# SonyCSLParis/audio-metrics

Hardware: AMD Instinct MI355X
Metric: evaluate() embeddings/sec (FAD+KD+PRDC), 2×100k CLAP-512 sets, 1/2/4/8 GPUs (higher is better)
Workload: dtype f32

## Files before the change

### audio-metrics_amd/csrc/pairwise_common.h

```cpp
#pragma once
#include "am_common.h"
#include "tile_engine.h"
#include <stdlib.h>

namespace am {

constexpr int EV_DEFAULT = EV_RSRC | EV_FRAGDB | EV_EARLY;
constexpr int WIDE_TILE_ROWS = 256;

#ifdef AM_DEV_KNOBS
static int env_int(const char* name, int dflt) {
    const char* v = getenv(name);
    return v ? atoi(v) : dflt;
}
static int engine_variant() {
    static const int v = env_int("AM_ENGINE_VARIANT", EV_DEFAULT);
    return v;
}
#else
static constexpr int env_int(const char*, int dflt) { return dflt; }
static constexpr int engine_variant() { return EV_DEFAULT; }
#endif

struct WorkItem {
// ... 141 lines not shown
}

constexpr unsigned FAST_COUNTED = 0x80000000u;
constexpr unsigned FAST_BOTH = 0x80000000u;
constexpr int FAST_ROW_OVERFLOW = 0x40000000;
constexpr unsigned FAST_HOLE = 0xffffffffu;

__device__ __forceinline__ unsigned long long lanes_le(float a, float b) { return __builtin_amdgcn_fcmpf(a, b, 5); }
__device__ __forceinline__ unsigned long long lanes_ge(float a, float b) { return __builtin_amdgcn_fcmpf(a, b, 3); }
__device__ __forceinline__ unsigned long long lanes_lt(float a, float b) { return __builtin_amdgcn_fcmpf(a, b, 4); }

template <int KCAP, class Lane = LaneInfo, int TBX = TB, int MT = 2>
struct KnnFastEpilogue {
    static constexpr int NWAVES = TBX == WIDE_TILE_ROWS ? 8 : 4;
    static constexpr int NT = Lane::NT;
    static constexpr bool ACC_INIT = Lane::ACC_INIT;
    const float* qnorm;
    const float* thr;
    int64_t n, pblock;
    float* aux;
    uint2* wgq;
    float* wgv;
    int wq;
    int wcap;
    uint2* shq;
    float* shv;
    int* qn;
    int shcap;
    uint2* ovq;
    float* ovv;
// ... 37 lines not shown
    }
    __device__ __forceinline__ void aux_issue(int, int64_t qtile) {
        if (L.tid < TBX) {
            const int64_t j = qtile * TBX + L.tid;
            aux_n = j < n ? qnorm[j] : INFINITY;
            aux_t = j < n ? __hip_atomic_load(thr + j, __ATOMIC_RELAXED, __HIP_MEMORY_SCOPE_AGENT) : -INFINITY;
        }
    }
    __device__ __forceinline__ void aux_commit(int t) {
        if (L.tid < TBX) {
            aux[(t & 1) * 2 * TBX + L.tid] = ACC_INIT ? aux_n * idsc : aux_n;
            aux[(t & 1) * 2 * TBX + TBX + L.tid] = ACC_INIT ? aux_t * idsc : aux_t;
        }
    }
    __device__ __forceinline__ f32x16 acc_init(int t, int mt) const {
        const float* a = aux + (t & 1) * 2 * TBX + L.wm * (MT * 32) + L.h * 4 + mt * 32;
        f32x16 c;
#pragma unroll
        for (int g4 = 0; g4 < 4; ++g4) {
            const f32x4 v = *reinterpret_cast<const f32x4*>(a + g4 * 8);
            c[g4 * 4 + 0] = v.x; c[g4 * 4 + 1] = v.y; c[g4 * 4 + 2] = v.z; c[g4 * 4 + 3] = v.w;
        }
        return c;
    }
    __device__ __forceinline__ void finish(int t, int64_t qtile, f32x16 (&acc)[MT][NT]) {
        const float* a = aux + (t & 1) * 2 * TBX + L.wm * (MT * 32) + L.h * 4;
        const bool mirror = qtile != pblock;
#ifdef AM_DEV_KNOBS
        if constexpr (TBX == WIDE_TILE_ROWS) {
            if (g_wide_dbg & 2) return;
        }
#endif
        const unsigned jbase = (unsigned)(qtile * TBX) + L.wm * (MT * 32) + L.h * 4;
        if constexpr (ACC_INIT) {
            float xsm[NT];
#pragma unroll
            for (int nt = 0; nt < NT; ++nt) xsm[nt] = mirror ? xs[nt] : INFINITY;
#pragma unroll
            for (int mt = 0; mt < MT; ++mt) {
                f32x4 tqs[4];
#pragma unroll
                for (int g4 = 0; g4 < 4; ++g4) tqs[g4] = *reinterpret_cast<const f32x4*>(a + TBX + mt * 32 + g4 * 8);
#pragma unroll
                for (int nt = 0; nt < NT; ++nt) {
                    float amax4[4], wmax4[4];
#pragma unroll
                    for (int g4 = 0; g4 < 4; ++g4) {
                        float am = -INFINITY, wm = -INFINITY;
#pragma unroll
                        for (int e = 0; e < 4; ++e) {
                            am = fmaxf(am, acc[mt][nt][g4 * 4 + e]);
                            wm = fmaxf(wm, acc[mt][nt][g4 * 4 + e] - tqs[g4][e]);
                        }
                        amax4[g4] = am;
                        wmax4[g4] = wm;
                    }
                    const float amax = fmaxf(fmaxf(amax4[0], amax4[1]), fmaxf(amax4[2], amax4[3]));
// ... 8 lines not shown
#endif
#pragma unroll
                    for (int g4 = 0; g4 < 4; ++g4) {
                        if ((lanes_le(fmaf(dsc, amax4[g4], xn[nt]), pl) | lanes_ge(wmax4[g4], xsm[nt])) == 0ull) continue;
#pragma unroll
                        for (int e = 0; e < 4; ++e) {
                            const int reg = g4 * 4 + e;
                            const float u = fmaf(dsc, acc[mt][nt][reg], xn[nt]);
                            const float w = acc[mt][nt][reg] - tqs[g4][e];
                            const unsigned long long sel = lanes_le(u, pl) | lanes_ge(w, xsm[nt]);
                            if (sel != 0ull) {
                                const bool own = u <= pl, mir = w >= xsm[nt];
                                const int below = __builtin_amdgcn_mbcnt_hi((unsigned)(sel >> 32), __builtin_amdgcn_mbcnt_lo((unsigned)sel, 0u));
                                const int slot = wq + below;
                                wq += __popcll(sel);
                                const unsigned j = jbase + mt * 32 + g4 * 8 + e;
#ifdef AM_DEV_KNOBS
                                if (TBX == WIDE_TILE_ROWS && (g_wide_dbg & 32)) continue;
#endif
                                if (own || mir) store_entry(slot, own ? prow[nt] : j, own ? j : prow[nt], own && mir, u);
                            }
                        }
                    }
                    const float vmin = tmin <= pl ? fmaxf(tmin, 0.f) : INFINITY;
#ifdef AM_DEV_KNOBS
                    if (TBX == WIDE_TILE_ROWS && (g_wide_dbg & 64)) continue;
#endif
                    if (lanes_lt(vmin, best[nt][KCAP - 1]) != 0ull) list_insert<KCAP>(best[nt], vmin);
                }
            }
            return;
        }
        const float mthr = mirror ? 0.f : -INFINITY;
#pragma unroll
        for (int mt = 0; mt < MT; ++mt) {
            f32x4 yn[4], tq[4];
#pragma unroll
            for (int g4 = 0; g4 < 4; ++g4) {
                yn[g4] = *reinterpret_cast<const f32x4*>(a + mt * 32 + g4 * 8);
                tq[g4] = *reinterpret_cast<const f32x4*>(a + TBX + mt * 32 + g4 * 8);
            }
#pragma unroll
            for (int nt = 0; nt < NT; ++nt) {
                float tmin4[4], marg4[4];
#pragma unroll
                for (int g4 = 0; g4 < 4; ++g4) {
                    float tm = INFINITY, mg = INFINITY;
#pragma unroll
                    for (int e = 0; e < 4; ++e) {
                        const float t = fmaf(dsc, acc[mt][nt][g4 * 4 + e], yn[g4][e]);
                        tm = fminf(tm, t);
                        mg = fminf(mg, t - tq[g4][e]);
                    }
                    tmin4[g4] = tm + xn[nt];
                    marg4[g4] = mg + xn[nt];
// ... 8 lines not shown
                }
#endif
#pragma unroll
                for (int g4 = 0; g4 < 4; ++g4) {
                    if ((lanes_le(tmin4[g4], pl) | lanes_le(marg4[g4], mthr)) == 0ull) continue;
#pragma unroll
                    for (int e = 0; e < 4; ++e) {
                        const int reg = g4 * 4 + e;
                        const float u = fmaf(dsc, acc[mt][nt][reg], xn[nt] + yn[g4][e]);
                        const bool own = u <= pl, mir = mirror && u <= tq[g4][e];
                        const unsigned long long sel = lanes_le(u, pl) | (mirror ? lanes_le(u, tq[g4][e]) : 0ull);
                        if (sel != 0ull) {
                            const int below = __builtin_amdgcn_mbcnt_hi((unsigned)(sel >> 32), __builtin_amdgcn_mbcnt_lo((unsigned)sel, 0u));
                            const int slot = wq + below;
                            wq += __popcll(sel);
                            const unsigned j = jbase + mt * 32 + g4 * 8 + e;
#ifdef AM_DEV_KNOBS
                            if (TBX == WIDE_TILE_ROWS && (g_wide_dbg & 32)) continue;
#endif
                            if (own || mir) store_entry(slot, own ? prow[nt] : j, own ? j : prow[nt], own && mir, u);
                        }
                    }
                }
                const float vmin = tmin <= pl ? fmaxf(tmin, 0.f) : INFINITY;
#ifdef AM_DEV_KNOBS
                if (TBX == WIDE_TILE_ROWS && (g_wide_dbg & 64)) continue;
#endif
                if (lanes_lt(vmin, best[nt][KCAP - 1]) != 0ull) list_insert<KCAP>(best[nt], vmin);
            }
        }
    }
// ... 38 lines not shown
```

### audio-metrics_amd/csrc/pairwise_pstat.hip

```cpp
#include "wide_kernels.h"
#include "pstat_engine.h"

namespace am {

template <int KSLABS>
struct PstatEng {
    using Lane = PLane;
    static constexpr int LDS_WORDS = pstat_lds_words(KSLABS);
    template <class TileMap, class Epi>
    static __device__ __forceinline__ void run(const float* Q, int64_t nq, int64_t ldq, const TileMap& tm, const float* P, int64_t np,
                                               int64_t ldp, int64_t prow0, int ntiles, int, float* lds, Lane& L, Epi& epi) {
        pstat_pipeline<KSLABS>(Q, nq, ldq, tm, P, np, ldp, prow0, ntiles, lds, L, epi);
    }
};

template <int KSLABS>
struct Pstat64Eng {
    using Lane = P64Lane;
    static constexpr int LDS_WORDS = pstat64_lds_words();
    template <class TileMap, class Epi>
    static __device__ __forceinline__ void run(const float* Q, int64_t nq, int64_t ldq, const TileMap& tm, const float* P, int64_t np,
                                               int64_t ldp, int64_t prow0, int ntiles, int, float* lds, Lane& L, Epi& epi) {
        pstat64_pipeline<KSLABS>(Q, nq, ldq, tm, P, np, ldp, prow0, ntiles, lds, L, epi);
    }
};

template <int KSLABS, bool WANT_MIN>
__global__ void __launch_bounds__(PTHREADS, 1)
cross_pstat_kernel(const float* __restrict__ Rb, int64_t Nr, int64_t ldr, const float* __restrict__ rnorm,
                   const float* __restrict__ rthr, const float* __restrict__ Cb, int64_t Nc, int64_t ldc,
                   const float* __restrict__ cnorm, const float* __restrict__ cthr, int Dh, int nchunks, int grp_rows,
                   const unsigned* __restrict__ maxn, unsigned* __restrict__ rmin_approx, unsigned* __restrict__ row_any,
                   unsigned* __restrict__ row_cover, int32_t* __restrict__ col_count, uint2* __restrict__ wgq, int qcap,
                   int* __restrict__ wgq_count, uint2* __restrict__ items, uint2* __restrict__ ovq, int* __restrict__ ov_count,
                   int ovcap, int* __restrict__ fail, float fc) {
    cross_wide_body<PstatEng<KSLABS>, WANT_MIN>(Rb, Nr, ldr, rnorm, rthr, Cb, Nc, ldc, cnorm, cthr, Dh, nchunks, grp_rows, maxn, rmin_approx,
                                                row_any, row_cover, col_count, wgq, qcap, wgq_count, items, ovq, ov_count, ovcap, fail, fc);
}

template <int KSLABS, int KCAP>
__global__ void __launch_bounds__(PTHREADS, 1)
knn_pstat_kernel(const float* __restrict__ Xb, int64_t N, int64_t ldh, const float* __restrict__ xnorm, float* thr, int Dh,
                 int win_tiles, int nwin, int per_win, int k1, const unsigned* __restrict__ maxn, float* __restrict__ partial,
                 int* __restrict__ cnt, int cap, uint2* __restrict__ wgq, float* __restrict__ wgv, int qcap,
                 int* __restrict__ wgq_count, int part, int nparts, float fc, uint2* __restrict__ ovq, float* __restrict__ ovv,
                 unsigned long long* __restrict__ ovn, int ovcap, const int* __restrict__ skip, int* __restrict__ region_counter) {
    knn_wide_body<PstatEng<KSLABS>, KCAP>(Xb, N, ldh, xnorm, thr, Dh, win_tiles, nwin, per_win, k1, maxn, partial, cnt, cap, wgq, wgv, qcap,
                                          wgq_count, part, nparts, fc, ovq, ovv, ovn, ovcap, skip, region_counter);
}

template <int KSLABS, bool WANT_MIN>
__global__ void __launch_bounds__(P64_THREADS, 2)
cross_pstat64_kernel(const float* __restrict__ Rb, int64_t Nr, int64_t ldr, const float* __restrict__ rnorm,
                     const float* __restrict__ rthr, const float* __restrict__ Cb, int64_t Nc, int64_t ldc,
                     const float* __restrict__ cnorm, const float* __restrict__ cthr, int Dh, int nchunks, int grp_rows,
                     const unsigned* __restrict__ maxn, unsigned* __restrict__ rmin_approx, unsigned* __restrict__ row_any,
                     unsigned* __restrict__ row_cover, int32_t* __restrict__ col_count, uint2* __restrict__ wgq, int qcap,
                     int* __restrict__ wgq_count, uint2* __restrict__ items, uint2* __restrict__ ovq, int* __restrict__ ov_count,
                     int ovcap, int* __restrict__ fail, float fc) {
    cross_wide_body<Pstat64Eng<KSLABS>, WANT_MIN>(Rb, Nr, ldr, rnorm, rthr, Cb, Nc, ldc, cnorm, cthr, Dh, nchunks, grp_rows, maxn, rmin_approx,
                                                  row_any, row_cover, col_count, wgq, qcap, wgq_count, items, ovq, ov_count, ovcap, fail, fc);
}
// ... 36 lines not shown
    AM_HIP_TRY(set_pstat_dev_symbols(st));
#endif
    hipLaunchKernelGGL((cross_pstat64_kernel<KSLABS, WANT_MIN>), dim3(blocks), dim3(P64_THREADS), lds_bytes, st, Rb, Nr, ldr, rnorm, rthr, Cb,
                       Nc, ldc, cnorm, cthr, Dh, nchunks, grp_rows, maxn, rmin_approx, row_any, row_cover, col_count, wgq, qcap,
                       wgq_count, items, ovq, ov_count, ovcap, fail, fc);
    AM_LAUNCH_CHECK();
    return AM_OK;
}

template <int KSLABS, bool WANT_MIN>
static int launch_cross_pstat_t(unsigned blocks, const float* Rb, int64_t Nr, int64_t ldr, const float* rnorm, const float* rthr,
                                const float* Cb, int64_t Nc, int64_t ldc, const float* cnorm, const float* cthr, int Dh, int nchunks,
                                int grp_rows, const unsigned* maxn, unsigned* rmin_approx, unsigned* row_any, unsigned* row_cover,
                                int32_t* col_count, uint2* wgq, int qcap, int* wgq_count, uint2* items, uint2* ovq, int* ov_count,
                                int ovcap, int* fail, float fc, hipStream_t st) {
    constexpr size_t lds_bytes = wide_cross_lds_bytes<PstatEng<KSLABS>>();
    AM_HIP_TRY(ensure_dynamic_lds(reinterpret_cast<const void*>(&cross_pstat_kernel<KSLABS, WANT_MIN>), (int)lds_bytes));
#ifdef AM_DEV_KNOBS
    AM_HIP_TRY(set_pstat_dev_symbols(st));
#endif
    hipLaunchKernelGGL((cross_pstat_kernel<KSLABS, WANT_MIN>), dim3(blocks), dim3(PTHREADS), lds_bytes, st, Rb, Nr, ldr, rnorm, rthr, Cb, Nc,
                       ldc, cnorm, cthr, Dh, nchunks, grp_rows, maxn, rmin_approx, row_any, row_cover, col_count, wgq, qcap, wgq_count,
                       items, ovq, ov_count, ovcap, fail, fc);
    AM_LAUNCH_CHECK();
    return AM_OK;
}

int launch_cross_pstat(bool want_min, unsigned blocks, const float* Rb, int64_t Nr, int64_t ldr, const float* rnorm, const float* rthr,
                       const float* Cb, int64_t Nc, int64_t ldc, const float* cnorm, const float* cthr, int Dh, int nchunks,
                       int grp_rows, const unsigned* maxn, unsigned* rmin_approx, unsigned* row_any, unsigned* row_cover,
                       int32_t* col_count, uint2* wgq, int qcap, int* wgq_count, uint2* items, uint2* ovq, int* ov_count, int ovcap,
// ... 37 lines not shown
#ifdef AM_DEV_KNOBS
    AM_HIP_TRY(set_pstat_dev_symbols(st));
#endif
    hipLaunchKernelGGL((knn_pstat64_kernel<KSLABS, KCAP>), dim3(nwg), dim3(P64_THREADS), lds_bytes, st, Xb, N, ldh, xnorm, thr, Dh, win_tiles,
                       nwin, per_win, k1, maxn, partial, cnt, cap, wgq, wgv, qcap, wgq_count, part, nparts, fc, ovq, ovv, ovn, ovcap, skip,
                       region_counter);
    AM_LAUNCH_CHECK();
    return AM_OK;
}

template <int KSLABS, int KCAP>
static int launch_knn_pstat_t(unsigned nwg, const float* Xb, int64_t N, int64_t ldh, const float* xnorm, float* thr, int Dh,
                              int win_tiles, int nwin, int per_win, int k1, const unsigned* maxn, float* partial, int* cnt, int cap,
                              uint2* wgq, float* wgv, int qcap, int* wgq_count, int part, int nparts, float fc, uint2* ovq,
                              float* ovv, unsigned long long* ovn, int ovcap, const int* skip, int* region_counter, hipStream_t st) {
    constexpr size_t lds_bytes = knn_wide_lds_bytes<PstatEng<KSLABS>>();
    AM_HIP_TRY(ensure_dynamic_lds(reinterpret_cast<const void*>(&knn_pstat_kernel<KSLABS, KCAP>), (int)lds_bytes));
#ifdef AM_DEV_KNOBS
    AM_HIP_TRY(set_pstat_dev_symbols(st));
#endif
    hipLaunchKernelGGL((knn_pstat_kernel<KSLABS, KCAP>), dim3(nwg), dim3(PTHREADS), lds_bytes, st, Xb, N, ldh, xnorm, thr, Dh, win_tiles,
                       nwin, per_win, k1, maxn, partial, cnt, cap, wgq, wgv, qcap, wgq_count, part, nparts, fc, ovq, ovv, ovn, ovcap, skip,
                       region_counter);
    AM_LAUNCH_CHECK();
    return AM_OK;
}

int launch_knn_pstat(int kcap, unsigned nwg, const float* Xb, int64_t N, int64_t ldh, const float* xnorm, float* thr, int Dh,
                     int win_tiles, int nwin, int per_win, int k1, const unsigned* maxn, float* partial, int* cnt, int cap,
                     uint2* wgq, float* wgv, int qcap, int* wgq_count, int part, int nparts, float fc, uint2* ovq, float* ovv,
                     unsigned long long* ovn, int ovcap, const int* skip, int* region_counter, hipStream_t st) {
// ... 32 lines not shown
```

### audio-metrics_amd/csrc/pstat_engine.h

```cpp
#pragma once
#include "wide_engine.h"

namespace am {

constexpr int PQ_ROWS = 128;
constexpr int PSTAGE_WORDS = PQ_ROWS * WROW;
constexpr int PRING = 4;
constexpr int PTHREADS = 512;
constexpr int PREG_SLABS = 6;
constexpr int pstat_lds_slabs(int kslabs) { return kslabs > PREG_SLABS ? kslabs - PREG_SLABS : 0; }
constexpr int pstat_lds_words(int kslabs) { return PRING * PSTAGE_WORDS + pstat_lds_slabs(kslabs) * WTB * WROW; }

struct PLane {
    static constexpr int NT = 1;
    static constexpr int MT = 4;
    static constexpr int WAVES = 8;
    static constexpr int LISTS = 2;
    static constexpr bool ACC_INIT = true;
    int tid, lane, wave, wm, r, h;
    __device__ __forceinline__ PLane() {
        tid = threadIdx.x;
        lane = tid & 63;
        wave = tid >> 6;
        wm = 0;
        r = lane & 31;
        h = lane >> 5;
    }
    __device__ __forceinline__ int prow(int) const { return wave * 32 + r; }
    __device__ __forceinline__ int list_slot() const { return h; }
};

template <int N>
__device__ __forceinline__ void pstat_wait() {
// ... 130 lines not shown
                if constexpr (Epi::ACC_INIT) {
                    if (u + 1 < units) {
                        L.wm = second ? 0 : 1;
#pragma unroll
                        for (int m = 0; m < 4; ++m) acc[m][0] = epi.acc_init((u + 1) >> 1, m);
                    }
                }
                __builtin_amdgcn_sched_barrier(0);
            }
        }
    }
    __builtin_amdgcn_s_waitcnt(0x0F70);
    __syncthreads();
}

constexpr int P64_THREADS = 256;
constexpr int P64_QROWS = 64;
constexpr int P64_STAGE_WORDS = P64_QROWS * WROW;
constexpr int P64_MAX_SLABS = 2;
constexpr int pstat64_lds_words() { return PRING * P64_STAGE_WORDS; }

struct P64Lane {
    static constexpr int NT = 2;
    static constexpr int MT = 2;
    static constexpr int WAVES = 4;
    static constexpr int LISTS = 2;
    static constexpr bool ACC_INIT = true;
    int tid, lane, wave, wm, r, h;
    __device__ __forceinline__ P64Lane() {
        tid = threadIdx.x;
        lane = tid & 63;
        wave = tid >> 6;
        wm = 0;
        r = lane & 31;
        h = lane >> 5;
    }
    __device__ __forceinline__ int prow(int nt) const { return wave * 64 + nt * 32 + r; }
    __device__ __forceinline__ int list_slot() const { return h; }
};

template <int KSLABS, class TileMap, class Epi>
__device__ __forceinline__ void pstat64_pipeline(const float* __restrict__ Q, int64_t nq, int64_t ldq, const TileMap& tmap,
// ... 132 lines not shown
```

### audio-metrics_amd/csrc/tile_engine.h

```cpp
#pragma once
#include <hip/hip_runtime.h>
#include <type_traits>

namespace am {

typedef float f32x16 __attribute__((ext_vector_type(16)));
typedef float f32x4 __attribute__((ext_vector_type(4)));

constexpr int TB = 128;
constexpr int BK = 32;
constexpr int LDK = 36;
constexpr int TILE_FLOATS = TB * LDK;
constexpr int STAGE_FLOATS = 2 * TILE_FLOATS;
constexpr int ENGINE_LDS_FLOATS = 2 * STAGE_FLOATS;
constexpr int ENGINE_THREADS = 256;

struct LaneInfo {
    static constexpr int NT = 2;
    static constexpr bool ACC_INIT = false;
    int tid, lane, wm, wn, r, h;
    __device__ __forceinline__ LaneInfo() {
        tid = threadIdx.x;
        lane = tid & 63;
        const int wave = tid >> 6;
        wm = wave >> 1;
        wn = wave & 1;
        r = lane & 31;
        h = lane >> 5;
    }
};

__device__ __forceinline__ f32x4 load_k4(const float* __restrict__ row, int k, int D) {
    f32x4 v = {0.f, 0.f, 0.f, 0.f};
    if (row != nullptr && k < D) {
// ... 563 lines not shown
```

### audio-metrics_amd/csrc/wide_engine.h

```cpp
#pragma once
#include "tile_engine.h"
#include <type_traits>

namespace am {

constexpr int WTB = 256;
constexpr int WTHREADS = 512;
constexpr int WROW = 32;
constexpr int WTILE_WORDS = WTB * WROW;
constexpr int WSTAGE_WORDS = 2 * WTILE_WORDS;
constexpr int WENGINE_LDS_WORDS = 2 * WSTAGE_WORDS;

struct WLane {
    static constexpr int NT = 2;
    static constexpr int MT = 4;
    static constexpr int WAVES = 8;
    static constexpr int LISTS = 4;
    static constexpr bool ACC_INIT = false;
    int tid, lane, wave, wm, wn, r, h;
    __device__ __forceinline__ WLane() {
        tid = threadIdx.x;
        lane = tid & 63;
        wave = tid >> 6;
        wm = wave >> 2;
        wn = wave & 3;
        r = lane & 31;
        h = lane >> 5;
    }
    __device__ __forceinline__ int prow(int nt) const { return wn * 64 + nt * 32 + r; }
    __device__ __forceinline__ int list_slot() const { return wm * 2 + h; }
};

__device__ __forceinline__ TileRsrc make_wide_rsrc(const float* base, int64_t ld, int64_t n_rows, int64_t row0, int dbg_bit = 1) {
// ... 169 lines not shown
```

### audio-metrics_amd/csrc/wide_kernels.h

```cpp
#pragma once
#include "pairwise_common.h"
#include "wide_engine.h"
#include <algorithm>

namespace am {

constexpr int WIDE_AUX_WORDS = 6 * WTB;
constexpr int WIDE_RAW_WORDS = 4 * WTB;
template <class Eng> constexpr size_t wide_cross_lds_bytes() { return (Eng::LDS_WORDS + WIDE_AUX_WORDS + WIDE_RAW_WORDS) * sizeof(float) + 16; }

template <class Lane>
struct CrossWideEpilogue {
    static constexpr int NT = Lane::NT;
    static constexpr int MT = Lane::MT;
    static constexpr bool ACC_INIT = Lane::ACC_INIT;
    const float* qnorm;
    const float* qthr;
    int64_t nq;
    float fc, rnmax_c;
    float* aux;
    int32_t* col_count;
    uint2* wgq;
    int* qn;
    int qcap;
    uint2* ovq;
    int* ov_count;
    int ovcap;
    int* fail;
    float dsc, idsc;
// ... 3 lines not shown
    bool rowok[NT], anyf[NT], covf[NT];
    float aux_n, aux_hi;
    const Lane& L;

    __device__ __forceinline__ CrossWideEpilogue(const Lane& l) : L(l) {}
    __device__ __forceinline__ void push(int64_t i, unsigned jflag) {
        const int slot = atomicAdd(qn, 1);
        if (slot < qcap) {
            wgq[slot] = make_uint2((unsigned)i, jflag);
        } else if (*reinterpret_cast<volatile int*>(fail) == 0) {
            const unsigned s2 = atomicAdd(reinterpret_cast<unsigned*>(ov_count), 1u);
            if (s2 < (unsigned)ovcap) ovq[s2] = make_uint2((unsigned)i, jflag);
            else *fail = 1;
        }
    }
    __device__ __forceinline__ void aux_issue(int, int64_t qtile) {
        if (L.tid < WTB) {
            const int64_t j = qtile * WTB + L.tid;
            const bool in = j < nq;
            aux_n = in ? qnorm[j] : INFINITY;
            aux_hi = in ? qthr[j] : -INFINITY;
        }
    }
    __device__ __forceinline__ void aux_commit(int t) {
        if (L.tid < WTB) {
            float* d = aux + (t & 1) * 3 * WTB + L.tid;
            const bool in = aux_hi > -INFINITY;
            const float e = fmaf(fc, aux_n, rnmax_c);
            d[0] = ACC_INIT ? aux_n * idsc : aux_n;
            d[WTB] = in ? (ACC_INIT ? (aux_hi + e) * idsc : aux_hi + e) : (ACC_INIT ? INFINITY : -INFINITY);
            d[2 * WTB] = in ? aux_hi - e : -INFINITY;
        }
    }
    __device__ __forceinline__ f32x16 acc_init(int t, int mt) const {
        const float* a = aux + (t & 1) * 3 * WTB + L.wm * (MT * 32) + L.h * 4 + mt * 32;
        f32x16 c;
#pragma unroll
        for (int g4 = 0; g4 < 4; ++g4) {
            const f32x4 v = *reinterpret_cast<const f32x4*>(a + g4 * 8);
            c[g4 * 4 + 0] = v.x; c[g4 * 4 + 1] = v.y; c[g4 * 4 + 2] = v.z; c[g4 * 4 + 3] = v.w;
        }
        return c;
    }
    template <bool WANT_MIN, bool NEED_ANY>
    __device__ __forceinline__ void finish_impl(int t, int64_t qtile, f32x16 (&acc)[MT][NT]) {
        const float* a = aux + (t & 1) * 3 * WTB + L.wm * (MT * 32) + L.h * 4;
        const int64_t jbase = qtile * WTB + L.wm * (MT * 32) + L.h * 4;
#ifdef AM_DEV_KNOBS
        if (g_wide_dbg & 2) return;
#endif
        if constexpr (ACC_INIT) {
#pragma unroll
            for (int mt = 0; mt < MT; ++mt) {
                f32x4 ths[4];
                if constexpr (NEED_ANY) {
#pragma unroll
                    for (int g4 = 0; g4 < 4; ++g4) ths[g4] = *reinterpret_cast<const f32x4*>(a + WTB + mt * 32 + g4 * 8);
                }
#pragma unroll
                for (int nt = 0; nt < NT; ++nt) {
                    float amax4[4], wmax4[4];
#pragma unroll
                    for (int g4 = 0; g4 < 4; ++g4) {
                        float am = -INFINITY, wmx = -INFINITY;
#pragma unroll
                        for (int e = 0; e < 4; ++e) {
                            am = fmaxf(am, acc[mt][nt][g4 * 4 + e]);
                            if constexpr (NEED_ANY) wmx = fmaxf(wmx, acc[mt][nt][g4 * 4 + e] - ths[g4][e]);
                        }
                        amax4[g4] = am;
                        wmax4[g4] = wmx;
                    }
                    const float tmin = fmaf(dsc, fmaxf(fmaxf(amax4[0], amax4[1]), fmaxf(amax4[2], amax4[3])), xn[nt]);
                    if constexpr (WANT_MIN) m[nt] = fminf(m[nt], fmaxf(tmin, 0.f));
                    const float prow_thr = WANT_MIN ? fmaxf(thi[nt], m[nt] + e2[nt]) : thi[nt];
                    {
                        unsigned long long hit = lanes_le(tmin, prow_thr);
                        if constexpr (NEED_ANY) hit |= lanes_ge(fmaxf(fmaxf(wmax4[0], wmax4[1]), fmaxf(wmax4[2], wmax4[3])), xsn[nt]);
                        if (hit == 0ull) continue;
#ifdef AM_DEV_KNOBS
                        if (g_wide_dbg & 16) continue;
#endif
                    }
                    const float* alo = a + 2 * WTB + mt * 32;
#pragma unroll
                    for (int g4 = 0; g4 < 4; ++g4) {
                        const bool row_hit = lanes_le(fmaf(dsc, amax4[g4], xn[nt]), prow_thr) != 0ull;
                        bool any_hit = false;
                        if constexpr (NEED_ANY) any_hit = lanes_ge(wmax4[g4], xsn[nt]) != 0ull;
#ifdef AM_DEV_KNOBS
                        if (g_wide_dbg & 8) any_hit = false;
#endif
                        if (!(row_hit || any_hit)) continue;
#pragma unroll
                        for (int e = 0; e < 4; ++e) {
                            const int reg = g4 * 4 + e;
                            const float u = fmaf(dsc, acc[mt][nt][reg], xn[nt]);
                            const int64_t j = jbase + mt * 32 + g4 * 8 + e;
                            bool sure = false, want = false;
                            if (row_hit) {
                                const unsigned long long mask = lanes_lt(u, tlo[nt]);
                                sure = u < tlo[nt];
                                if (mask != 0ull && L.lane == 0) {
                                    const int lo = __popcll(mask & 0xffffffffull);
                                    const int hi = __popcll(mask >> 32);
                                    if (lo) atomicAdd(col_count + j - L.h * 4, lo);
                                    if (hi) atomicAdd(col_count + j - L.h * 4 + 4, hi);
                                }
                                covf[nt] = covf[nt] || sure;
                                want = !sure && u <= thi[nt];
                                if constexpr (WANT_MIN) want = want || u <= m[nt] + e2[nt];
                            }
                            if constexpr (NEED_ANY) {
                                if (acc[mt][nt][reg] - ths[g4][e] >= xsn[nt]) {
                                    if (u < alo[g4 * 8 + e]) {
                                        anyf[nt] = true;
                                        xsn[nt] = INFINITY;
                                    } else {
                                        want = true;
                                    }
                                }
                            }
                            if (want) push(prow[nt], (unsigned)j | (sure ? FAST_COUNTED : 0u));
                        }
                    }
                }
            }
            return;
        }
#pragma unroll
        for (int mt = 0; mt < MT; ++mt) {
            f32x4 yn[4], th[4];
#pragma unroll
            for (int g4 = 0; g4 < 4; ++g4) {
                yn[g4] = *reinterpret_cast<const f32x4*>(a + mt * 32 + g4 * 8);
                if constexpr (NEED_ANY) th[g4] = *reinterpret_cast<const f32x4*>(a + WTB + mt * 32 + g4 * 8);
            }
#pragma unroll
            for (int nt = 0; nt < NT; ++nt) {
                float tmin4[4], marg4[4];
#pragma unroll
                for (int g4 = 0; g4 < 4; ++g4) {
                    float tm = INFINITY, mg = INFINITY;
#pragma unroll
                    for (int e = 0; e < 4; ++e) {
                        const float t = fmaf(dsc, acc[mt][nt][g4 * 4 + e], yn[g4][e]);
                        tm = fminf(tm, t);
                        if constexpr (NEED_ANY) mg = fminf(mg, t - th[g4][e]);
                    }
                    tmin4[g4] = tm + xn[nt];
                    if constexpr (NEED_ANY) marg4[g4] = mg + xn[nt];
                }
                const float tmin = fminf(fminf(tmin4[0], tmin4[1]), fminf(tmin4[2], tmin4[3]));
                if constexpr (WANT_MIN) m[nt] = fminf(m[nt], fmaxf(tmin, 0.f));
                const float prow_thr = WANT_MIN ? fmaxf(thi[nt], m[nt] + e2[nt]) : thi[nt];
                {
                    unsigned long long hit = lanes_le(tmin, prow_thr);
                    if constexpr (NEED_ANY) hit |= lanes_le(fminf(fminf(marg4[0], marg4[1]), fminf(marg4[2], marg4[3])), athr[nt]);
                    if (hit == 0ull) continue;
#ifdef AM_DEV_KNOBS
                    if (g_wide_dbg & 16) continue;
#endif
                }
                const float* alo = a + 2 * WTB + mt * 32;
#pragma unroll
                for (int g4 = 0; g4 < 4; ++g4) {
                    const bool row_hit = lanes_le(tmin4[g4], prow_thr) != 0ull;
                    bool any_hit = false;
                    if constexpr (NEED_ANY) any_hit = lanes_le(marg4[g4], athr[nt]) != 0ull;
#ifdef AM_DEV_KNOBS
                    if (g_wide_dbg & 8) any_hit = false;
#endif
                    if (!(row_hit || any_hit)) continue;
#pragma unroll
                    for (int e = 0; e < 4; ++e) {
                        const int reg = g4 * 4 + e;
                        const float u = fmaf(dsc, acc[mt][nt][reg], xn[nt] + yn[g4][e]);
                        const int64_t j = jbase + mt * 32 + g4 * 8 + e;
                        bool sure = false, want = false;
                        if (row_hit) {
                            sure = u < tlo[nt];
                            const unsigned long long mask = lanes_lt(u, tlo[nt]);
                            if (mask != 0ull && L.lane == 0) {
                                const int lo = __popcll(mask & 0xffffffffull);
                                const int hi = __popcll(mask >> 32);
                                if (lo) atomicAdd(col_count + j - L.h * 4, lo);
                                if (hi) atomicAdd(col_count + j - L.h * 4 + 4, hi);
                            }
                            covf[nt] = covf[nt] || sure;
                            want = !sure && u <= thi[nt];
                            if constexpr (WANT_MIN) want = want || u <= m[nt] + e2[nt];
                        }
                        if constexpr (NEED_ANY) {
                            if (!anyf[nt] && u <= th[g4][e]) {
                                if (u < alo[g4 * 8 + e]) {
                                    anyf[nt] = true;
                                    athr[nt] = -INFINITY;
                                } else {
                                    want = true;
                                }
                            }
                        }
                        if (want) push(prow[nt], (unsigned)j | (sure ? FAST_COUNTED : 0u));
                    }
                }
            }
        }
    }
};

// ... 98 lines not shown
        epi.athr[nt] = epi.anyf[nt] ? -INFINITY : 0.f;
        epi.covf[nt] = false;
    }
#ifdef AM_DEV_KNOBS
    if (g_wide_dbg & 4) {
        CrossWideShim<Lane, WANT_MIN, false> quick{epi};
        Eng::run(Cb, Nc, ldc, WideTiles{w.qtile0}, Rb, Nr, ldr, prow0, w.ntiles, Dh, lds, L, quick);
    } else
#endif
    {
        CrossWideShim<Lane, WANT_MIN, true> shim{epi};
        Eng::run(Cb, Nc, ldc, WideTiles{w.qtile0}, Rb, Nr, ldr, prow0, w.ntiles, Dh, lds, L, shim);
    }
#pragma unroll
    for (int nt = 0; nt < Lane::NT; ++nt) {
        const float mn = fminf(epi.m[nt], __shfl_xor(epi.m[nt], 32));
        const int other = __shfl_xor((int)epi.anyf[nt], 32);
        const int other_c = __shfl_xor((int)epi.covf[nt], 32);
        const bool any = epi.anyf[nt] || other != 0;
        const bool cov = epi.covf[nt] || other_c != 0;
        if (L.h == 0 && epi.rowok[nt]) {
            if constexpr (WANT_MIN) atomicMin(rmin_approx + epi.prow[nt], __float_as_uint(mn));
            if (any) atomicOr(row_any + epi.prow[nt], 1u);
            if (cov) atomicOr(row_cover + epi.prow[nt], 1u);
        }
    }
    __syncthreads();
    if (L.tid == 0) {
        const int n = *qn < qcap ? *qn : qcap, nb = (n + 63) / 64;
        wgq_count[blockIdx.x] = n;
        qn[0] = n;
        qn[1] = nb > 0 ? atomicAdd(ov_count + 2, nb) : 0;
    }
// ... 127 lines not shown
```

Baseline: 8.893 million.

## Add 16x16x32 f16 MFMA pstat pipeline for cross kernel without min tracking

```diff
diff --git a/audio-metrics_amd/csrc/pairwise_common.h b/audio-metrics_amd/csrc/pairwise_common.h
--- a/audio-metrics_amd/csrc/pairwise_common.h
+++ b/audio-metrics_amd/csrc/pairwise_common.h
@@ -179,6 +179,7 @@
 struct KnnFastEpilogue {
     static constexpr int NWAVES = TBX == WIDE_TILE_ROWS ? 8 : 4;
     static constexpr int NT = Lane::NT;
+    static constexpr int QT = Lane::QT, GS = Lane::GSTRIDE;
     static constexpr bool ACC_INIT = Lane::ACC_INIT;
     const float* qnorm;
     const float* thr;
@@ -246,24 +247,24 @@
         }
     }
     __device__ __forceinline__ f32x16 acc_init(int t, int mt) const {
-        const float* a = aux + (t & 1) * 2 * TBX + L.wm * (MT * 32) + L.h * 4 + mt * 32;
+        const float* a = aux + (t & 1) * 2 * TBX + L.wm * (MT * QT) + L.h * 4 + mt * QT;
         f32x16 c;
 #pragma unroll
         for (int g4 = 0; g4 < 4; ++g4) {
-            const f32x4 v = *reinterpret_cast<const f32x4*>(a + g4 * 8);
+            const f32x4 v = *reinterpret_cast<const f32x4*>(a + g4 * GS);
             c[g4 * 4 + 0] = v.x; c[g4 * 4 + 1] = v.y; c[g4 * 4 + 2] = v.z; c[g4 * 4 + 3] = v.w;
         }
         return c;
     }
     __device__ __forceinline__ void finish(int t, int64_t qtile, f32x16 (&acc)[MT][NT]) {
-        const float* a = aux + (t & 1) * 2 * TBX + L.wm * (MT * 32) + L.h * 4;
+        const float* a = aux + (t & 1) * 2 * TBX + L.wm * (MT * QT) + L.h * 4;
         const bool mirror = qtile != pblock;
 #ifdef AM_DEV_KNOBS
         if constexpr (TBX == WIDE_TILE_ROWS) {
             if (g_wide_dbg & 2) return;
         }
 #endif
-        const unsigned jbase = (unsigned)(qtile * TBX) + L.wm * (MT * 32) + L.h * 4;
+        const unsigned jbase = (unsigned)(qtile * TBX) + L.wm * (MT * QT) + L.h * 4;
         if constexpr (ACC_INIT) {
             float xsm[NT];
 #pragma unroll
@@ -272,7 +273,7 @@
             for (int mt = 0; mt < MT; ++mt) {
                 f32x4 tqs[4];
 #pragma unroll
-                for (int g4 = 0; g4 < 4; ++g4) tqs[g4] = *reinterpret_cast<const f32x4*>(a + TBX + mt * 32 + g4 * 8);
+                for (int g4 = 0; g4 < 4; ++g4) tqs[g4] = *reinterpret_cast<const f32x4*>(a + TBX + mt * QT + g4 * GS);
 #pragma unroll
                 for (int nt = 0; nt < NT; ++nt) {
                     float amax4[4], wmax4[4];
@@ -311,7 +312,7 @@
                                 const int below = __builtin_amdgcn_mbcnt_hi((unsigned)(sel >> 32), __builtin_amdgcn_mbcnt_lo((unsigned)sel, 0u));
                                 const int slot = wq + below;
                                 wq += __popcll(sel);
-                                const unsigned j = jbase + mt * 32 + g4 * 8 + e;
+                                const unsigned j = jbase + mt * QT + g4 * GS + e;
 #ifdef AM_DEV_KNOBS
                                 if (TBX == WIDE_TILE_ROWS && (g_wide_dbg & 32)) continue;
 #endif
@@ -334,8 +335,8 @@
             f32x4 yn[4], tq[4];
 #pragma unroll
             for (int g4 = 0; g4 < 4; ++g4) {
-                yn[g4] = *reinterpret_cast<const f32x4*>(a + mt * 32 + g4 * 8);
-                tq[g4] = *reinterpret_cast<const f32x4*>(a + TBX + mt * 32 + g4 * 8);
+                yn[g4] = *reinterpret_cast<const f32x4*>(a + mt * QT + g4 * GS);
+                tq[g4] = *reinterpret_cast<const f32x4*>(a + TBX + mt * QT + g4 * GS);
             }
 #pragma unroll
             for (int nt = 0; nt < NT; ++nt) {
@@ -374,7 +375,7 @@
                             const int below = __builtin_amdgcn_mbcnt_hi((unsigned)(sel >> 32), __builtin_amdgcn_mbcnt_lo((unsigned)sel, 0u));
                             const int slot = wq + below;
                             wq += __popcll(sel);
-                            const unsigned j = jbase + mt * 32 + g4 * 8 + e;
+                            const unsigned j = jbase + mt * QT + g4 * GS + e;
 #ifdef AM_DEV_KNOBS
                             if (TBX == WIDE_TILE_ROWS && (g_wide_dbg & 32)) continue;
 #endif
diff --git a/audio-metrics_amd/csrc/pairwise_pstat.hip b/audio-metrics_amd/csrc/pairwise_pstat.hip
--- a/audio-metrics_amd/csrc/pairwise_pstat.hip
+++ b/audio-metrics_amd/csrc/pairwise_pstat.hip
@@ -1,18 +1,24 @@
 #include "wide_kernels.h"
 #include "pstat_engine.h"
+#include <type_traits>
 
 namespace am {
 
-template <int KSLABS>
+template <int KSLABS, bool S16 = false>
 struct PstatEng {
-    using Lane = PLane;
+    using Lane = std::conditional_t<S16, P16Lane, PLane>;
     static constexpr int LDS_WORDS = pstat_lds_words(KSLABS);
+    static constexpr bool cross16(bool want_min) { return KSLABS == 8 && !want_min; }
+    static constexpr bool knn16(int) { return false; }
     template <class TileMap, class Epi>
     static __device__ __forceinline__ void run(const float* Q, int64_t nq, int64_t ldq, const TileMap& tm, const float* P, int64_t np,
                                                int64_t ldp, int64_t prow0, int ntiles, int, float* lds, Lane& L, Epi& epi) {
-        pstat_pipeline<KSLABS>(Q, nq, ldq, tm, P, np, ldp, prow0, ntiles, lds, L, epi);
+        if constexpr (S16) pstat16_pipeline<KSLABS>(Q, nq, ldq, tm, P, np, ldp, prow0, ntiles, lds, L, epi);
+        else pstat_pipeline<KSLABS>(Q, nq, ldq, tm, P, np, ldp, prow0, ntiles, lds, L, epi);
     }
 };
+template <int KSLABS, bool WANT_MIN> using CrossPstatEng = PstatEng<KSLABS, PstatEng<KSLABS>::cross16(WANT_MIN)>;
+template <int KSLABS, int KCAP> using KnnPstatEng = PstatEng<KSLABS, PstatEng<KSLABS>::knn16(KCAP)>;
 
 template <int KSLABS>
 struct Pstat64Eng {
@@ -34,7 +40,7 @@
                    unsigned* __restrict__ row_cover, int32_t* __restrict__ col_count, uint2* __restrict__ wgq, int qcap,
                    int* __restrict__ wgq_count, uint2* __restrict__ items, uint2* __restrict__ ovq, int* __restrict__ ov_count,
                    int ovcap, int* __restrict__ fail, float fc) {
-    cross_wide_body<PstatEng<KSLABS>, WANT_MIN>(Rb, Nr, ldr, rnorm, rthr, Cb, Nc, ldc, cnorm, cthr, Dh, nchunks, grp_rows, maxn, rmin_approx,
+    cross_wide_body<CrossPstatEng<KSLABS, WANT_MIN>, WANT_MIN>(Rb, Nr, ldr, rnorm, rthr, Cb, Nc, ldc, cnorm, cthr, Dh, nchunks, grp_rows, maxn, rmin_approx,
                                                 row_any, row_cover, col_count, wgq, qcap, wgq_count, items, ovq, ov_count, ovcap, fail, fc);
 }
 
@@ -45,7 +51,7 @@
                  int* __restrict__ cnt, int cap, uint2* __restrict__ wgq, float* __restrict__ wgv, int qcap,
                  int* __restrict__ wgq_count, int part, int nparts, float fc, uint2* __restrict__ ovq, float* __restrict__ ovv,
                  unsigned long long* __restrict__ ovn, int ovcap, const int* __restrict__ skip, int* __restrict__ region_counter) {
-    knn_wide_body<PstatEng<KSLABS>, KCAP>(Xb, N, ldh, xnorm, thr, Dh, win_tiles, nwin, per_win, k1, maxn, partial, cnt, cap, wgq, wgv, qcap,
+    knn_wide_body<KnnPstatEng<KSLABS, KCAP>, KCAP>(Xb, N, ldh, xnorm, thr, Dh, win_tiles, nwin, per_win, k1, maxn, partial, cnt, cap, wgq, wgv, qcap,
                                           wgq_count, part, nparts, fc, ovq, ovv, ovn, ovcap, skip, region_counter);
 }
 
@@ -112,7 +118,7 @@
                                 int grp_rows, const unsigned* maxn, unsigned* rmin_approx, unsigned* row_any, unsigned* row_cover,
                                 int32_t* col_count, uint2* wgq, int qcap, int* wgq_count, uint2* items, uint2* ovq, int* ov_count,
                                 int ovcap, int* fail, float fc, hipStream_t st) {
-    constexpr size_t lds_bytes = wide_cross_lds_bytes<PstatEng<KSLABS>>();
+    constexpr size_t lds_bytes = wide_cross_lds_bytes<CrossPstatEng<KSLABS, WANT_MIN>>();
     AM_HIP_TRY(ensure_dynamic_lds(reinterpret_cast<const void*>(&cross_pstat_kernel<KSLABS, WANT_MIN>), (int)lds_bytes));
 #ifdef AM_DEV_KNOBS
     AM_HIP_TRY(set_pstat_dev_symbols(st));
@@ -180,7 +186,7 @@
                               int win_tiles, int nwin, int per_win, int k1, const unsigned* maxn, float* partial, int* cnt, int cap,
                               uint2* wgq, float* wgv, int qcap, int* wgq_count, int part, int nparts, float fc, uint2* ovq,
                               float* ovv, unsigned long long* ovn, int ovcap, const int* skip, int* region_counter, hipStream_t st) {
-    constexpr size_t lds_bytes = knn_wide_lds_bytes<PstatEng<KSLABS>>();
+    constexpr size_t lds_bytes = knn_wide_lds_bytes<KnnPstatEng<KSLABS, KCAP>>();
     AM_HIP_TRY(ensure_dynamic_lds(reinterpret_cast<const void*>(&knn_pstat_kernel<KSLABS, KCAP>), (int)lds_bytes));
 #ifdef AM_DEV_KNOBS
     AM_HIP_TRY(set_pstat_dev_symbols(st));
diff --git a/audio-metrics_amd/csrc/pstat_engine.h b/audio-metrics_amd/csrc/pstat_engine.h
--- a/audio-metrics_amd/csrc/pstat_engine.h
+++ b/audio-metrics_amd/csrc/pstat_engine.h
@@ -17,6 +17,7 @@
     static constexpr int WAVES = 8;
     static constexpr int LISTS = 2;
     static constexpr bool ACC_INIT = true;
+    static constexpr int GSTRIDE = 8, GROUPS = 2, QT = 32;
     int tid, lane, wave, wm, r, h;
     __device__ __forceinline__ PLane() {
         tid = threadIdx.x;
@@ -177,6 +178,185 @@
     __syncthreads();
 }
 
+struct P16Lane {
+    static constexpr int NT = 2;
+    static constexpr int MT = 2;
+    static constexpr int WAVES = 8;
+    static constexpr int LISTS = 4;
+    static constexpr bool ACC_INIT = true;
+    static constexpr int GSTRIDE = 16, GROUPS = 4, QT = 64;
+    int tid, lane, wave, wm, r, h;
+    __device__ __forceinline__ P16Lane() {
+        tid = threadIdx.x;
+        lane = tid & 63;
+        wave = tid >> 6;
+        wm = 0;
+        r = lane & 15;
+        h = lane >> 4;
+    }
+    __device__ __forceinline__ int prow(int nt) const { return wave * 32 + nt * 16 + r; }
+    __device__ __forceinline__ int list_slot() const { return h; }
+};
+
+template <int KSLABS, class TileMap, class Epi>
+__device__ __forceinline__ void pstat16_pipeline(const float* __restrict__ Q, int64_t nq, int64_t ldq, const TileMap& tmap,
+                                                 const float* __restrict__ P, int64_t np, int64_t ldp, int64_t prow0, int ntiles,
+                                                 float* __restrict__ lds, P16Lane& L, Epi& epi) {
+    static_assert(KSLABS >= 1 && KSLABS <= 8, "P fragments of at most 512 f16 per row fit the register file");
+    static_assert(Epi::ACC_INIT, "the epilogues of this engine start their accumulators at the column norm");
+    constexpr int KREG = KSLABS < PREG_SLABS ? KSLABS : PREG_SLABS;
+    constexpr int KLDS = KSLABS - KREG;
+    constexpr int KSTEPS = KREG * 2;
+    constexpr int PIECES = 2;
+    constexpr int DEPTH = 3;
+    const int wave = __builtin_amdgcn_readfirstlane(L.wave);
+
+    f32x4 pf[2][KSTEPS];
+    {
+        const TileRsrc prs = make_wide_rsrc(P, ldp, np, prow0, 0);
+#pragma unroll
+        for (int nt = 0; nt < 2; ++nt) {
+            const unsigned vop = (unsigned)(((int64_t)(wave * 32 + nt * 16 + L.r) * ldp + L.h * 4) * 4);
+#pragma unroll
+            for (int s = 0; s < KSTEPS; ++s)
+                pf[nt][s] = __builtin_bit_cast(f32x4, __builtin_amdgcn_raw_buffer_load_b128(prs.rsrc, (int)vop, s * 64, 0));
+        }
+        const int lr8 = L.lane >> 3, s8 = L.lane & 7;
+#pragma unroll
+        for (int sl = 0; sl < KLDS; ++sl)
+#pragma unroll
+            for (int i = 0; i < 4; ++i) {
+                const int row = wave * 32 + i * 8 + lr8;
+                const unsigned vo = (unsigned)(((int64_t)row * ldp + (s8 ^ ((row >> 1) & 7)) * 4) * 4);
+                lds_direct_b128(prs, lds + PRING * PSTAGE_WORDS + sl * WTB * WROW + (wave * 32 + i * 8) * WROW, vo, (unsigned)((KREG + sl) * 128));
+            }
+    }
+    const float* plds = lds + PRING * PSTAGE_WORDS + wave * 32 * WROW;
+
+    const int lr = L.lane >> 3, slot8 = L.lane & 7;
+    const unsigned voq0 = (unsigned)(((int64_t)lr * ldq + (slot8 ^ ((lr >> 1) & 7)) * 4) * 4);
+    const unsigned odd_soff = (unsigned)((int64_t)8 * ldq * 4);
+    const unsigned wave_soff = (unsigned)((int64_t)wave * 16 * ldq * 4), half_soff = (unsigned)((int64_t)PQ_ROWS * ldq * 4);
+    const int64_t q_tiles_total = (nq + WTB - 1) / WTB;
+    auto qtile_of = [&](int t) -> int64_t { return t < ntiles ? tmap(t) : q_tiles_total; };
+    int ft = 0, fh = 0, fk = 0, fslot = 0;
+    TileRsrc qrs = make_wide_rsrc(Q, ldq, nq, qtile_of(0) * WTB);
+    auto fetch_stage = [&](int i) {
+        float* dst = lds + fslot * PSTAGE_WORDS + (wave * 2 + i) * 8 * WROW;
+        lds_direct_b128(qrs, dst, i == 0 ? voq0 : (voq0 ^ 64u), (unsigned)(fk * 128) + (fh ? half_soff : 0u) + wave_soff + (i == 0 ? 0u : odd_soff));
+    };
+    auto advance_fetch = [&]() {
+        fslot = (fslot + 1) & (PRING - 1);
+        if (++fk == KSLABS) {
+            fk = 0;
+            fh ^= 1;
+            if (fh == 0) {
+                ++ft;
+                qrs = make_wide_rsrc(Q, ldq, nq, qtile_of(ft) * WTB);
+            }
+        }
+    };
+
+    const int sw = (L.r >> 1) & 7;
+    int coff[2];
+#pragma unroll
+    for (int c = 0; c < 2; ++c) coff[c] = L.r * WROW + ((4 * c + L.h) ^ sw) * 4;
+    auto qfrag = [&](int ring_slot, int c, int mt) -> f32x4 {
+        return *reinterpret_cast<const f32x4*>(lds + ring_slot * PSTAGE_WORDS + mt * 16 * WROW + coff[c]);
+    };
+    auto pfrag_lds = [&](int step, int nt) -> f32x4 {
+        return *reinterpret_cast<const f32x4*>(plds + (step / 2 - KREG) * WTB * WROW + nt * 16 * WROW + coff[step & 1]);
+    };
+
+    f32x16 acc[2][2];
+
+#pragma unroll
+    for (int g = 0; g < DEPTH; ++g) {
+        fetch_stage(0);
+        fetch_stage(1);
+        advance_fetch();
+    }
+    epi.aux_issue(0, qtile_of(0));
+    __builtin_amdgcn_s_waitcnt(0x0F70);
+    epi.aux_commit(0);
+    pstat_wait<0>();
+    __builtin_amdgcn_s_barrier();
+
+    f32x4 q[4];
+    f32x4 pl[2][2];
+    int slot = 0;
+#pragma unroll
+    for (int m = 0; m < 4; ++m) q[m] = qfrag(0, 0, m);
+    L.wm = 0;
+#pragma unroll
+    for (int m = 0; m < 2; ++m) {
+        const f32x16 c0 = epi.acc_init(0, m);
+        acc[m][0] = c0;
+        acc[m][1] = c0;
+    }
+    const int units = 2 * ntiles;
+    for (int u = 0; u < units; ++u) {
+        const int t = u >> 1;
+        const bool second = (u & 1) != 0;
+#pragma unroll
+        for (int ks = 0; ks < KSLABS; ++ks) {
+            const bool last_stage = ks == KSLABS - 1;
+            const int next_slot = (slot + 1) & (PRING - 1);
+            if (last_stage && second && t + 1 < ntiles) epi.aux_issue(t + 1, qtile_of(t + 1));
+#pragma unroll
+            for (int c = 0; c < 2; ++c) {
+                const int step = ks * 2 + c;
+                if (KLDS > 0 && step + 1 >= KSTEPS && step + 1 < KSLABS * 2) {
+                    pl[(step + 1) & 1][0] = pfrag_lds(step + 1, 0);
+                    pl[(step + 1) & 1][1] = pfrag_lds(step + 1, 1);
+                }
+                const f32x4 pb0 = step < KSTEPS ? pf[0][step < KSTEPS ? step : 0] : pl[step & 1][0];
+                const f32x4 pb1 = step < KSTEPS ? pf[1][step < KSTEPS ? step : 0] : pl[step & 1][1];
+#pragma unroll
+                for (int mt = 0; mt < 8; ++mt) {
+                    const int m = mt >> 2, t4 = (mt & 3) * 4;
+#pragma unroll
+                    for (int nt = 0; nt < 2; ++nt) {
+                        f32x4 a = {acc[m][nt][t4], acc[m][nt][t4 + 1], acc[m][nt][t4 + 2], acc[m][nt][t4 + 3]};
+                        a = __builtin_amdgcn_mfma_f32_16x16x32_f16(__builtin_bit_cast(f16x8, q[mt & 3]), __builtin_bit_cast(f16x8, nt == 0 ? pb0 : pb1), a, 0, 0, 0);
+                        acc[m][nt][t4] = a.x; acc[m][nt][t4 + 1] = a.y; acc[m][nt][t4 + 2] = a.z; acc[m][nt][t4 + 3] = a.w;
+                    }
+                    if (mt < 4) q[mt & 3] = qfrag(slot, c, mt + 4);
+                    else if (c == 0) q[mt & 3] = qfrag(slot, 1, mt - 4);
+                    else if (!last_stage) q[mt & 3] = qfrag(next_slot, 0, mt - 4);
+                    if (mt == 1) fetch_stage(c);
+                    __builtin_amdgcn_sched_barrier(0);
+                }
+            }
+            advance_fetch();
+            if (last_stage) {
+                L.wm = second ? 1 : 0;
+                epi.finish(t, qtile_of(t), acc);
+                if (second && t + 1 < ntiles) epi.aux_commit(t + 1);
+            }
+            pstat_wait<PIECES>();
+            __builtin_amdgcn_s_barrier();
+            slot = next_slot;
+            if (last_stage) {
+#pragma unroll
+                for (int m = 0; m < 4; ++m) q[m] = qfrag(slot, 0, m);
+                if (u + 1 < units) {
+                    L.wm = second ? 0 : 1;
+#pragma unroll
+                    for (int m = 0; m < 2; ++m) {
+                        const f32x16 c0 = epi.acc_init((u + 1) >> 1, m);
+                        acc[m][0] = c0;
+                        acc[m][1] = c0;
+                    }
+                }
+                __builtin_amdgcn_sched_barrier(0);
+            }
+        }
+    }
+    __builtin_amdgcn_s_waitcnt(0x0F70);
+    __syncthreads();
+}
+
 constexpr int P64_THREADS = 256;
 constexpr int P64_QROWS = 64;
 constexpr int P64_STAGE_WORDS = P64_QROWS * WROW;
@@ -189,6 +369,7 @@
     static constexpr int WAVES = 4;
     static constexpr int LISTS = 2;
     static constexpr bool ACC_INIT = true;
+    static constexpr int GSTRIDE = 8, GROUPS = 2, QT = 32;
     int tid, lane, wave, wm, r, h;
     __device__ __forceinline__ P64Lane() {
         tid = threadIdx.x;
diff --git a/audio-metrics_amd/csrc/tile_engine.h b/audio-metrics_amd/csrc/tile_engine.h
--- a/audio-metrics_amd/csrc/tile_engine.h
+++ b/audio-metrics_amd/csrc/tile_engine.h
@@ -18,6 +18,7 @@
 struct LaneInfo {
     static constexpr int NT = 2;
     static constexpr bool ACC_INIT = false;
+    static constexpr int GSTRIDE = 8, GROUPS = 2, QT = 32;
     int tid, lane, wm, wn, r, h;
     __device__ __forceinline__ LaneInfo() {
         tid = threadIdx.x;
diff --git a/audio-metrics_amd/csrc/wide_engine.h b/audio-metrics_amd/csrc/wide_engine.h
--- a/audio-metrics_amd/csrc/wide_engine.h
+++ b/audio-metrics_amd/csrc/wide_engine.h
@@ -17,6 +17,7 @@
     static constexpr int WAVES = 8;
     static constexpr int LISTS = 4;
     static constexpr bool ACC_INIT = false;
+    static constexpr int GSTRIDE = 8, GROUPS = 2, QT = 32;
     int tid, lane, wave, wm, wn, r, h;
     __device__ __forceinline__ WLane() {
         tid = threadIdx.x;
diff --git a/audio-metrics_amd/csrc/wide_kernels.h b/audio-metrics_amd/csrc/wide_kernels.h
--- a/audio-metrics_amd/csrc/wide_kernels.h
+++ b/audio-metrics_amd/csrc/wide_kernels.h
@@ -13,6 +13,7 @@
 struct CrossWideEpilogue {
     static constexpr int NT = Lane::NT;
     static constexpr int MT = Lane::MT;
+    static constexpr int QT = Lane::QT, GS = Lane::GSTRIDE;
     static constexpr bool ACC_INIT = Lane::ACC_INIT;
     const float* qnorm;
     const float* qthr;
@@ -46,6 +47,14 @@
             else *fail = 1;
         }
     }
+    __device__ __forceinline__ void count_columns(unsigned long long mask, int64_t j) {
+        constexpr int W = 64 / Lane::GROUPS;
+#pragma unroll
+        for (int q = 0; q < Lane::GROUPS; ++q) {
+            const int c = __popcll(q == Lane::GROUPS - 1 ? mask >> (q * W) : (mask >> (q * W)) & (~0ull >> (64 - W)));
+            if (c) atomicAdd(col_count + j - L.h * 4 + q * 4, c);
+        }
+    }
     __device__ __forceinline__ void aux_issue(int, int64_t qtile) {
         if (L.tid < WTB) {
             const int64_t j = qtile * WTB + L.tid;
@@ -65,19 +74,19 @@
         }
     }
     __device__ __forceinline__ f32x16 acc_init(int t, int mt) const {
-        const float* a = aux + (t & 1) * 3 * WTB + L.wm * (MT * 32) + L.h * 4 + mt * 32;
+        const float* a = aux + (t & 1) * 3 * WTB + L.wm * (MT * QT) + L.h * 4 + mt * QT;
         f32x16 c;
 #pragma unroll
         for (int g4 = 0; g4 < 4; ++g4) {
-            const f32x4 v = *reinterpret_cast<const f32x4*>(a + g4 * 8);
+            const f32x4 v = *reinterpret_cast<const f32x4*>(a + g4 * GS);
             c[g4 * 4 + 0] = v.x; c[g4 * 4 + 1] = v.y; c[g4 * 4 + 2] = v.z; c[g4 * 4 + 3] = v.w;
         }
         return c;
     }
     template <bool WANT_MIN, bool NEED_ANY>
     __device__ __forceinline__ void finish_impl(int t, int64_t qtile, f32x16 (&acc)[MT][NT]) {
-        const float* a = aux + (t & 1) * 3 * WTB + L.wm * (MT * 32) + L.h * 4;
-        const int64_t jbase = qtile * WTB + L.wm * (MT * 32) + L.h * 4;
+        const float* a = aux + (t & 1) * 3 * WTB + L.wm * (MT * QT) + L.h * 4;
+        const int64_t jbase = qtile * WTB + L.wm * (MT * QT) + L.h * 4;
 #ifdef AM_DEV_KNOBS
         if (g_wide_dbg & 2) return;
 #endif
@@ -87,7 +96,7 @@
                 f32x4 ths[4];
                 if constexpr (NEED_ANY) {
 #pragma unroll
-                    for (int g4 = 0; g4 < 4; ++g4) ths[g4] = *reinterpret_cast<const f32x4*>(a + WTB + mt * 32 + g4 * 8);
+                    for (int g4 = 0; g4 < 4; ++g4) ths[g4] = *reinterpret_cast<const f32x4*>(a + WTB + mt * QT + g4 * GS);
                 }
 #pragma unroll
                 for (int nt = 0; nt < NT; ++nt) {
@@ -114,7 +123,7 @@
                         if (g_wide_dbg & 16) continue;
 #endif
                     }
-                    const float* alo = a + 2 * WTB + mt * 32;
+                    const float* alo = a + 2 * WTB + mt * QT;
 #pragma unroll
                     for (int g4 = 0; g4 < 4; ++g4) {
                         const bool row_hit = lanes_le(fmaf(dsc, amax4[g4], xn[nt]), prow_thr) != 0ull;
@@ -128,24 +137,19 @@
                         for (int e = 0; e < 4; ++e) {
                             const int reg = g4 * 4 + e;
                             const float u = fmaf(dsc, acc[mt][nt][reg], xn[nt]);
-                            const int64_t j = jbase + mt * 32 + g4 * 8 + e;
+                            const int64_t j = jbase + mt * QT + g4 * GS + e;
                             bool sure = false, want = false;
                             if (row_hit) {
                                 const unsigned long long mask = lanes_lt(u, tlo[nt]);
                                 sure = u < tlo[nt];
-                                if (mask != 0ull && L.lane == 0) {
-                                    const int lo = __popcll(mask & 0xffffffffull);
-                                    const int hi = __popcll(mask >> 32);
-                                    if (lo) atomicAdd(col_count + j - L.h * 4, lo);
-                                    if (hi) atomicAdd(col_count + j - L.h * 4 + 4, hi);
-                                }
+                                if (mask != 0ull && L.lane == 0) count_columns(mask, j);
                                 covf[nt] = covf[nt] || sure;
                                 want = !sure && u <= thi[nt];
                                 if constexpr (WANT_MIN) want = want || u <= m[nt] + e2[nt];
                             }
                             if constexpr (NEED_ANY) {
                                 if (acc[mt][nt][reg] - ths[g4][e] >= xsn[nt]) {
-                                    if (u < alo[g4 * 8 + e]) {
+                                    if (u < alo[g4 * GS + e]) {
                                         anyf[nt] = true;
                                         xsn[nt] = INFINITY;
                                     } else {
@@ -165,8 +169,8 @@
             f32x4 yn[4], th[4];
 #pragma unroll
             for (int g4 = 0; g4 < 4; ++g4) {
-                yn[g4] = *reinterpret_cast<const f32x4*>(a + mt * 32 + g4 * 8);
-                if constexpr (NEED_ANY) th[g4] = *reinterpret_cast<const f32x4*>(a + WTB + mt * 32 + g4 * 8);
+                yn[g4] = *reinterpret_cast<const f32x4*>(a + mt * QT + g4 * GS);
+                if constexpr (NEED_ANY) th[g4] = *reinterpret_cast<const f32x4*>(a + WTB + mt * QT + g4 * GS);
             }
 #pragma unroll
             for (int nt = 0; nt < NT; ++nt) {
@@ -194,7 +198,7 @@
                     if (g_wide_dbg & 16) continue;
 #endif
                 }
-                const float* alo = a + 2 * WTB + mt * 32;
+                const float* alo = a + 2 * WTB + mt * QT;
 #pragma unroll
                 for (int g4 = 0; g4 < 4; ++g4) {
                     const bool row_hit = lanes_le(tmin4[g4], prow_thr) != 0ull;
@@ -208,24 +212,19 @@
                     for (int e = 0; e < 4; ++e) {
                         const int reg = g4 * 4 + e;
                         const float u = fmaf(dsc, acc[mt][nt][reg], xn[nt] + yn[g4][e]);
-                        const int64_t j = jbase + mt * 32 + g4 * 8 + e;
+                        const int64_t j = jbase + mt * QT + g4 * GS + e;
                         bool sure = false, want = false;
                         if (row_hit) {
                             sure = u < tlo[nt];
                             const unsigned long long mask = lanes_lt(u, tlo[nt]);
-                            if (mask != 0ull && L.lane == 0) {
-                                const int lo = __popcll(mask & 0xffffffffull);
-                                const int hi = __popcll(mask >> 32);
-                                if (lo) atomicAdd(col_count + j - L.h * 4, lo);
-                                if (hi) atomicAdd(col_count + j - L.h * 4 + 4, hi);
-                            }
+                            if (mask != 0ull && L.lane == 0) count_columns(mask, j);
                             covf[nt] = covf[nt] || sure;
                             want = !sure && u <= thi[nt];
                             if constexpr (WANT_MIN) want = want || u <= m[nt] + e2[nt];
                         }
                         if constexpr (NEED_ANY) {
                             if (!anyf[nt] && u <= th[g4][e]) {
-                                if (u < alo[g4 * 8 + e]) {
+                                if (u < alo[g4 * GS + e]) {
                                     anyf[nt] = true;
                                     athr[nt] = -INFINITY;
                                 } else {
@@ -354,9 +353,15 @@
     }
 #pragma unroll
     for (int nt = 0; nt < Lane::NT; ++nt) {
-        const float mn = fminf(epi.m[nt], __shfl_xor(epi.m[nt], 32));
-        const int other = __shfl_xor((int)epi.anyf[nt], 32);
-        const int other_c = __shfl_xor((int)epi.covf[nt], 32);
+        float mn = fminf(epi.m[nt], __shfl_xor(epi.m[nt], 32));
+        int other = __shfl_xor((int)epi.anyf[nt], 32);
+        int other_c = __shfl_xor((int)epi.covf[nt], 32);
+#pragma unroll
+        for (int off = 16; off >= 64 / Lane::GROUPS; off >>= 1) {
+            mn = fminf(mn, __shfl_xor(mn, off));
+            other |= __shfl_xor(other | (int)epi.anyf[nt], off);
+            other_c |= __shfl_xor(other_c | (int)epi.covf[nt], off);
+        }
         const bool any = epi.anyf[nt] || other != 0;
         const bool cov = epi.covf[nt] || other_c != 0;
         if (L.h == 0 && epi.rowok[nt]) {
```

Result: faster. 9.279 million, median of 6 (+4.3%).
